# lmdu/pyfastx

Measured on AMD Instinct MI355X. Metric: FASTA index build + 1M random 100bp subseq fetches, 3 Gbp plain FASTA per GPU (throughput of the whole step, stream resident in HBM), higher is better.
Workload: dtype u8; 1 GPU; configs[1]: synthetic 3.0 Gbp hg38-shaped plain FASTA per GPU (200 contigs, 60-col LF, soft-masked, N runs), index build + 1000000 random 100 bp intervals (50% '-' strand); parallelism=one GPU, the whole stream resident in its HBM

## Files before the change

pyfastx_amd/csrc/fx_kernels.hpp:

```cpp
#pragma once
#include <hip/hip_runtime.h>
#include <stdint.h>

namespace fx {

constexpr int BLOCK = 256;
constexpr int UNROLL = 8;
constexpr int CHUNK = 16;
constexpr int TILE = BLOCK * CHUNK * UNROLL;

__device__ __forceinline__ uint32_t zero_bytes(uint32_t x) {
    return ~(((x & 0x7F7F7F7Fu) + 0x7F7F7F7Fu) | x | 0x7F7F7F7Fu);
}
__device__ __forceinline__ uint32_t flags4(uint32_t t) { return __builtin_amdgcn_udot4(t, 0x08040201u, 0u, false) >> 7; }
__device__ __forceinline__ uint32_t eq_mask16(const uint4 &v, uint32_t pat) {
    uint32_t lo = __builtin_amdgcn_udot4(zero_bytes(v.x ^ pat), 0x08040201u, 0u, false);
    lo = __builtin_amdgcn_udot4(zero_bytes(v.y ^ pat), 0x80402010u, lo, false);
    uint32_t hi = __builtin_amdgcn_udot4(zero_bytes(v.z ^ pat), 0x08040201u, 0u, false);
    hi = __builtin_amdgcn_udot4(zero_bytes(v.w ^ pat), 0x80402010u, hi, false);
    return (lo >> 7) | (hi << 1);
}

__device__ __forceinline__ uint4 load16(const uint8_t *__restrict__ data, int64_t p, int64_t n) {
    if (p + CHUNK <= n) return *reinterpret_cast<const uint4 *>(data + p);
// ... 327 lines not shown
                    uint32_t word = w[0];
#pragma unroll
                    for (int k = 1; k < NW; ++k) word = (j >> 2) == k ? w[k] : word;
                    uint8_t c = (uint8_t)(word >> ((j & 3) * 8));
                    if ((fl & 1) && c >= 'a' && c <= 'z') c -= 32;
                    if (fl & 4) c = lut[c];
                    const int64_t o = r - skip;
                    out[(fl & 2) ? (take - 1 - o) : o] = c;
                }
                ++r;
            }
            rank += total;
        }
        if (ok) {
            int64_t got = rank - skip;
            got = got < 0 ? 0 : (got > take ? take : got);
            if ((fl & 2) && got < take && got > 0) {
                const int64_t delta = take - got;
                for (int64_t j0 = 0; j0 < got; j0 += G) {
                    const int64_t j = j0 + sub;
                    uint8_t c = 0;
                    if (j < got) c = out[delta + j];
                    if (j < got) out[j] = c;
                }
            }
            if (sub == 0 && q.out_len) q.out_len[i] = got;
        }
    }
}

template <int G, int NP, bool COAL = false>
__global__ __launch_bounds__(BLOCK) void k_fetch_lines(const uint8_t *__restrict__ data, int64_t gbase, int64_t n_bytes, FetchQ q, FastaTab tab,
                                                      int64_t nq, int flags_all, uint8_t *__restrict__ dst, int32_t *__restrict__ list,
                                                      int *__restrict__ list_n) {
    __shared__ uint8_t lut[256];
    constexpr int CO_CAP = 2048;
    __shared__ __attribute__((aligned(16))) uint32_t s_out[COAL ? BLOCK / 64 : 1][COAL ? (CO_CAP + 32) / 4 : 1];
    constexpr int TABCAP = 512;
    __shared__ int64_t s_boff[TABCAP], s_slen[TABCAP];
    __shared__ int32_t s_llen[TABCAP], s_en[TABCAP];
    const int64_t n_seq = tab.n_seq_dev ? (*tab.n_seq_dev < tab.n_seq ? (int64_t)*tab.n_seq_dev : tab.n_seq) : tab.n_seq;
    const bool tab_lds = n_seq <= TABCAP && n_seq > 0;
    build_comp_lut(lut);
    if (tab_lds)
        for (int r = threadIdx.x; r < (int)n_seq; r += BLOCK) {
            s_boff[r] = tab.boff[r]; s_slen[r] = tab.slen[r];
            const int64_t ll = tab.llen[r];
            s_llen[r] = ll > 0x7FFFFFFFll ? 0x7FFFFFFF : (int32_t)ll;
            s_en[r] = tab.elen[r] | (tab.norm[r] << 8);
        }
    __syncthreads();
    constexpr int QPW = 64 / G;
    const int lane = lane_id(), sub = lane & (G - 1), grp = lane / G;
    const int64_t wave = ((int64_t)blockIdx.x * BLOCK + threadIdx.x) >> 6;
    const int64_t nwaves = ((int64_t)gridDim.x * BLOCK) >> 6;
    int64_t d_id = 0, d_a = 0, d_b = 0, d_off = 0;
    int d_fl = flags_all;
    auto fetch_desc = [&](int64_t i) {
        if (i >= nq) return;
        d_id = q.seq_id[i]; d_a = q.start[i]; d_b = q.stop[i];
        d_off = q.dst_off[i];
        d_fl = q.qflags ? q.qflags[i] : flags_all;
    };
    fetch_desc(wave * QPW + grp);
    for (int64_t i0 = wave * QPW; i0 < nq; i0 += nwaves * QPW) {
        const int64_t i = i0 + grp;
        const bool live = i < nq;
        const int64_t id = d_id, a = d_a, b = d_b;
// ... 339 lines not shown
```

pyfastx_amd/csrc/fx_spanscan.hpp:

```cpp
#pragma once
#include "fx_kernels.hpp"

namespace fx {

#ifndef FX_GRAN
#define FX_GRAN 4096
#endif
constexpr int GRAN = FX_GRAN;
constexpr int GR_ROWS = GRAN / (64 * CHUNK);
constexpr int SPAN_GRANS = 65536 / GRAN;
constexpr int SPAN = GRAN * SPAN_GRANS;
constexpr uint32_t SP_NONE = 0xFFFFFFFFu;

struct GranOut { uint32_t n, h, first, last, v1, c1, v2, c2, ovf; };
struct __attribute__((aligned(16))) GranPk { uint32_t nh, fl, d1, d2; };
__device__ __forceinline__ GranPk gran_pack(const GranOut &o) {
    GranPk p;
    p.nh = o.n | (o.h << 16); p.fl = (o.first & 0xFFFFu) | (o.last << 16);
    p.d1 = o.v1 | (o.c1 << 16); p.d2 = o.v2 | (o.c2 << 16) | (o.ovf << 31);
    return p;
}
__device__ __forceinline__ GranOut gran_unpack(const GranPk &p) {
    GranOut o;
    o.n = p.nh & 0xFFFFu; o.h = p.nh >> 16;
// ... 284 lines not shown
    }
    Tri tot;
    tri_block_incl(gran_tri(go, (int64_t)blockIdx.x * CG + threadIdx.x, ngran, gbase), lds, &tot);
    if (threadIdx.x == 0) ct[blockIdx.x] = ChunkTot{tot.n, tot.h, tot.last, 0};
}

struct Tri32 { uint32_t n, h; int32_t last; };
__device__ __forceinline__ Tri32 tri32_block_incl(Tri32 v, uint32_t (*lds)[16], Tri32 *total) {
    const int w = threadIdx.x >> 6, l = lane_id(), nw = (blockDim.x + 63) >> 6;
#pragma unroll
    for (int d = 1; d < 64; d <<= 1) {
        const uint32_t a = __shfl_up(v.n, d, 64), b = __shfl_up(v.h, d, 64);
        const int32_t c = __shfl_up(v.last, d, 64);
        if (l >= d) { v.n += a; v.h += b; v.last = c > v.last ? c : v.last; }
    }
    __syncthreads();
    if (l == 63) { lds[0][w] = v.n; lds[1][w] = v.h; lds[2][w] = (uint32_t)v.last; }
    __syncthreads();
    Tri32 base{0, 0, -1}, tot{0, 0, -1};
    for (int i = 0; i < nw; ++i) {
        const uint32_t a = lds[0][i], b = lds[1][i];
        const int32_t c = (int32_t)lds[2][i];
        if (i < w) { base.n += a; base.h += b; base.last = c > base.last ? c : base.last; }
        tot.n += a; tot.h += b; tot.last = c > tot.last ? c : tot.last;
    }
    *total = tot;
    return Tri32{base.n + v.n, base.h + v.h, base.last > v.last ? base.last : v.last};
}

template <int CG>
__global__ __launch_bounds__(CG) void k_gran_prefix(const GranPk *__restrict__ go, int64_t ngran, int64_t gbase,
                                                            const ChunkTot *__restrict__ ct, Totals *__restrict__ tot,
                                                            int64_t *__restrict__ nl_prefix, int64_t *__restrict__ hdr_prefix,
                                                            int64_t *__restrict__ prevnl) {
    __shared__ Tri lds[CG / 64];
    __shared__ uint32_t lds32[3][16];
    Tri b{0, 0, -1};
    for (int64_t c = threadIdx.x; c < (int64_t)blockIdx.x; c += CG) { const ChunkTot t = ct[c]; b = tri_join(b, Tri{t.n, t.h, t.last}); }
    Tri base{0, 0, -1};
    if (blockIdx.x) tri_block_incl(b, lds, &base);
    const int64_t g = (int64_t)blockIdx.x * CG + threadIdx.x;
    Tri32 v{0, 0, -1};
    if (g < ngran) {
        const GranOut o = gran_unpack(go[g]);
        v = Tri32{o.n, o.h, o.n ? (int32_t)(threadIdx.x * GRAN + o.last) : -1};
    }
    Tri32 total;
    const Tri32 inc = tri32_block_incl(v, lds32, &total);
    const int64_t cstart = gbase + (int64_t)blockIdx.x * CG * GRAN;
    if (g < ngran) {
        nl_prefix[g] = base.n + (inc.n - v.n);
        hdr_prefix[g] = base.h + (inc.h - v.h);
        int32_t pm = __shfl_up(inc.last, 1, 64);
        if (lane_id() == 0) { pm = -1; for (int i = 0; i < (int)(threadIdx.x >> 6); ++i) { const int32_t c = (int32_t)lds32[2][i]; pm = c > pm ? c : pm; } }
        prevnl[g] = pm >= 0 ? cstart + pm : base.last;
    }
    if (blockIdx.x == gridDim.x - 1 && threadIdx.x == 0) {
        const int64_t tn = base.n + total.n, th = base.h + total.h, tl = total.last >= 0 ? cstart + total.last : base.last;
        nl_prefix[ngran] = tn; hdr_prefix[ngran] = th; prevnl[ngran] = tl;
        tot->n_nl = tn; tot->n_hdr = th; tot->last_nl = tl;
    }
}

struct ScanCtx {
    const uint8_t *data; int64_t n, gbase, ngran;
    const GranPk *go;
    const int64_t *nl_prefix, *hdr_prefix, *prevnl;
};

__device__ __forceinline__ int64_t next_nl(const ScanCtx &c, int64_t x) {
    const int64_t y = x + 1 - c.gbase;
    if (y > c.n) return -1;
    const int64_t g = y / GRAN;
    if (g < c.ngran) {
        const GranOut o = gran_unpack(c.go[g]);
        const int64_t gs = g * (int64_t)GRAN;
        if (o.n && gs + o.last >= y) {
            if (gs + o.first >= y) return c.gbase + gs + o.first;
            for (int64_t p = y & ~(int64_t)(CHUNK - 1); p < gs + GRAN; p += CHUNK) {
                const uint4 v = load16(c.data, p, c.n);
                uint32_t m = eq_mask16(v, 0x0A0A0A0Au);
                if (p < y) m &= 0xFFFFu << (y - p);
                if (m) return c.gbase + p + (__ffs(m) - 1);
                if (p + CHUNK > c.n) break;
            }
            return c.gbase + gs + o.last;
        }
    }
    const int64_t key = c.gbase + (g + 1) * (int64_t)GRAN;
    int64_t lo = g + 1, hi = c.ngran;
    if (lo >= hi || c.prevnl[c.ngran] < key) return -1;
    while (lo < hi) { const int64_t mid = (lo + hi) >> 1; if (c.prevnl[mid + 1] >= key) hi = mid; else lo = mid + 1; }
    return c.gbase + lo * (int64_t)GRAN + (c.go[lo].fl & 0xFFFFu);
// ... 281 lines not shown
            if (mism) atomicAdd(&rv.bad[r], mism);
            return;
        }
    }
    irr.g[atomicAdd(irr.count, 1u)] = (uint32_t)g;
}

__global__ __launch_bounds__(BLOCK) void k_gran_exact(ScanCtx x, RecView rv, int64_t cap, GranList irr, int is_last, int prev_byte) {
    const int lane = lane_id();
    const int64_t wave = ((int64_t)blockIdx.x * blockDim.x + threadIdx.x) >> 6;
    const int64_t nwaves = ((int64_t)gridDim.x * blockDim.x) >> 6;
    const int64_t cnt = *irr.count;
    int64_t i = wave, g = i < cnt ? irr.g[i] : 0;
    uint4 v[GR_ROWS];
    if (i < cnt) {
#pragma unroll
        for (int j = 0; j < GR_ROWS; ++j) v[j] = load16(x.data, g * (int64_t)GRAN + j * 1024 + lane * CHUNK, x.n);
    }
    for (; i < cnt; i += nwaves) {
        const int64_t gc = g, hb = x.hdr_prefix[gc];
        int64_t he = x.hdr_prefix[gc + 1];
        if (he > cap) he = cap;
        ExactMasks mk;
        exact_masks(x, v, is_last, prev_byte, gc, he > hb, mk);
        if (i + nwaves < cnt) {
            g = irr.g[i + nwaves];
#pragma unroll
            for (int j = 0; j < GR_ROWS; ++j) v[j] = load16(x.data, g * (int64_t)GRAN + j * 1024 + lane * CHUNK, x.n);
        }
        exact_rows(x, rv, cap, gc, hb, mk);
    }
}

__global__ __launch_bounds__(BLOCK) void k_fasta_finalize2(int64_t cap, FastaCols c, Totals *__restrict__ tot,
                                                          const uint8_t *__restrict__ data, int64_t n_bytes, int64_t gbase) {
    const int64_t *__restrict__ hdr = c.hoff, *__restrict__ hdr_line = c.hdr_line;
    const int64_t k = (int64_t)blockIdx.x * BLOCK + threadIdx.x;
    const int64_t n_hdr = tot->n_hdr < cap ? tot->n_hdr : cap;
    int64_t s = 0;
    if (k < n_hdr) {
        if (c.dlen[k] >= 0) {
            int64_t hn, Ln;
            if (k + 1 < n_hdr) { hn = hdr[k + 1]; Ln = hdr_line[k + 1]; }
            else               { hn = tot->last_nl + 1; Ln = tot->n_nl; }
            const int64_t nseq = Ln - hdr_line[k] - 1;
            const int64_t blen = hn - c.boff[k];
            s = blen - (int64_t)c.elen[k] * nseq;
            c.blen[k] = blen; c.slen[k] = s;
            const int norm = c.bad[k] > 1 ? 0 : 1;
            c.norm[k] = norm;
            int reg = line_regular(data, n_bytes, gbase, c.boff[k], blen, s, nseq > 0 ? c.llen[k] : 0, c.elen[k], norm);
            if (reg < 0) reg = c.bad[k] == 0;
            c.reg[k] = reg;
        } else { c.blen[k] = 0; c.slen[k] = 0; c.norm[k] = 1; c.reg[k] = 0; }
    }
    __shared__ unsigned long long blk;
    if (threadIdx.x == 0) blk = 0;
    __syncthreads();
    s = wave_sum64(s);
    if (lane_id() == 0 && s) atomicAdd(&blk, (unsigned long long)s);
    __syncthreads();
    if (threadIdx.x == 0 && blk) atomicAdd((unsigned long long *)&tot->seq_len, blk);
}

__global__ __launch_bounds__(BLOCK) void k_line_regular(const uint8_t *__restrict__ data, int64_t n_bytes, int64_t gbase, int64_t n,
                                                       const int64_t *__restrict__ boff, const int64_t *__restrict__ blen,
                                                       const int64_t *__restrict__ slen, const int64_t *__restrict__ llen,
                                                       const int32_t *__restrict__ elen, const int32_t *__restrict__ norm,
                                                       int32_t *__restrict__ reg) {
    const int64_t k = (int64_t)blockIdx.x * BLOCK + threadIdx.x;
    if (k < n) reg[k] = line_regular(data, n_bytes, gbase, boff[k], blen[k], slen[k], llen[k], elen[k], norm[k]) > 0 ? 1 : 0;
}

__device__ __forceinline__ int64_t prev_nl_wave(const ScanCtx &x, int64_t p) {
    const int64_t y = (p - x.gbase < x.n) ? p - x.gbase : x.n;
    if (y <= 0) return -1;
    const int64_t g = (y - 1) / GRAN;
    const int64_t a = g * (int64_t)GRAN + lane_id() * 64;
    unsigned long long m = 0;
#pragma unroll
    for (int i = 0; i < 4; ++i)
        if (a + i * CHUNK < y) m |= (unsigned long long)eq_mask16(load16(x.data, a + i * CHUNK, x.n), 0x0A0A0A0Au) << (16 * i);
    if (y - a < 64) m &= (y - a <= 0) ? 0ull : (~0ull >> (64 - (y - a)));
    const unsigned long long b = __ballot(m != 0);
    if (!b) return x.prevnl[g];
    const int l = 63 - __clzll(b);
    const int hi = __shfl((int)(m >> 32), l, 64), lo = __shfl((int)(m & 0xFFFFFFFFull), l, 64);
    const unsigned long long ml = ((unsigned long long)(unsigned int)hi << 32) | (unsigned int)lo;
    return x.gbase + g * (int64_t)GRAN + l * 64 + (63 - __clzll(ml));
}

constexpr int SUMM_BLOCK = 1024;
__device__ __forceinline__ DiffSet diffset_shfl_xor(const DiffSet &d, int m) {
    return DiffSet{(uint32_t)__shfl_xor((int)d.v1, m, 64), (uint32_t)__shfl_xor((int)d.c1, m, 64), (uint32_t)__shfl_xor((int)d.v2, m, 64),
                   (uint32_t)__shfl_xor((int)d.c2, m, 64), (uint32_t)__shfl_xor((int)d.ovf, m, 64)};
// ... 210 lines not shown
```

pyfastx_amd/csrc/fxgpu.hip:

```cpp
#include <hip/hip_runtime.h>
#include <zlib.h>
#include <fcntl.h>
#include <pthread.h>
#include <sched.h>
#include <sys/mman.h>
#include <sys/stat.h>
#include <unistd.h>

#include <algorithm>
#include <atomic>
#include <chrono>
#include <functional>
#include <map>
#include <memory>
#include <cstdarg>
#include <cstdio>
#include <cstdlib>
#include <cstring>
#include <mutex>
#include <string>
#include <thread>
#include <vector>

#include "../../include/fxgpu.h"
// ... 313 lines not shown
        (h)->prof.end((h)->stream);                                               \
    } while (0)
#define FX_LAUNCH_LDS(h, id, kern, grid, block, lds, ...)                         \
    do {                                                                          \
        (h)->prof.begin(id, (h)->stream);                                         \
        hipLaunchKernelGGL(kern, grid, block, lds, (h)->stream, __VA_ARGS__);     \
        (h)->prof.end((h)->stream);                                               \
    } while (0)

struct StageAsync;
static void stage_drop(fx_handle *h);
struct fx_handle {
    int device = 0;
    hipStream_t stream = nullptr;
    StageAsync *stage = nullptr;
    int stage_fd = -1;
    hipStream_t stream2 = nullptr;
    uint8_t *d_data = nullptr;
    uint8_t *d_alloc = nullptr;
    size_t blob_cap = 0;
    bool owns = false;
    int64_t n = 0;
    bool gz = false;
    int64_t base = 0;
    int prev_byte = '\n';
    bool is_last = true;
    int64_t n_nl = 0;
    bool scanned = false;
    int64_t ngran = 0;
    DevBuf<GranPk> gran;
    DevBuf<uint32_t> hdr_grans, irr_grans;
    DevBuf<ChunkTot> chunks;
    DevBuf<unsigned long long> ctl;
    Totals *pin_tot = nullptr;
    struct OneBox { int64_t off, blen, skip, take, dst_off, out_len; } *one_box = nullptr;
    uint8_t *one_out = nullptr;
    Mailbox *mb = nullptr;
    hipStream_t mb_stream = nullptr;
    unsigned long long mb_seq = 0;
    bool mb_running = false, mb_off = false;
    DevBuf<uint32_t> nm_table;
    DevBuf<int64_t> nm_off;
    uint64_t nm_mask = 0;
    int nm_kind = -1;
    DevBuf<int64_t> nl_prefix, hdr_prefix, prevnl;
    DevBuf<int64_t> hdr, fa_boff, fa_blen, fa_slen, fa_llen, fa_hdr_line;
    DevBuf<int32_t> fa_elen, fa_norm, fa_dlen, fa_name_len, fa_reg;
    DevBuf<uint32_t> fa_bad;
    int64_t n_hdr = 0, fa_seqlen = 0;
    bool fasta_built = false;
    bool build_pending = false;
    int pending_full_name = 0;
    DevBuf<uint32_t> comp_runs;
    int comp_gpw = 0;
    bool comp_runs_valid = false;
    DevBuf<int64_t> fq_name_off, fq_rlen, fq_soff, fq_qoff;
    DevBuf<int32_t> fq_name_len, fq_dlen, fq_qlen;
    DevBuf<FastqAcc> fq_acc;
    DevBuf<FqRun> fq_runs;
    DevBuf<FastqAcc> fq_acc_build;
    DevBuf<uint32_t> fq_rej;
    int64_t fq_comp_runs = 0, fq_comp_rejected = 0;
    bool fq_comp_valid = false;
    int64_t fq_comp_base[5] = {0, 0, 0, 0, 0};
    int fq_comp_minqs = 104, fq_comp_maxqs = 33;
    DevBuf<uint32_t> fq_lines;
    bool fq_by_lines = false;
// ... 1520 lines not shown
        if (rc) return rc;
        for (int64_t i = 0; i < m; ++i) {
            unsigned char c = buf[i];
            if (!(c == ' ' || (c >= 9 && c <= 13))) { *out = c; return FX_OK; }
        }
    }
    return FX_OK;
}


static ScanCtx scan_ctx(const fx_handle *h) {
    ScanCtx x;
    x.data = h->d_data; x.n = h->n; x.gbase = h->base; x.ngran = h->ngran;
    x.go = h->gran.p; x.nl_prefix = h->nl_prefix.p; x.hdr_prefix = h->hdr_prefix.p; x.prevnl = h->prevnl.p;
    return x;
}
static FastaCols fasta_cols(fx_handle *h) {
    FastaCols c;
    c.hoff = h->hdr.p; c.boff = h->fa_boff.p; c.blen = h->fa_blen.p; c.slen = h->fa_slen.p; c.llen = h->fa_llen.p;
    c.hdr_line = h->fa_hdr_line.p; c.elen = h->fa_elen.p; c.dlen = h->fa_dlen.p; c.name_len = h->fa_name_len.p;
    c.norm = h->fa_norm.p; c.bad = h->fa_bad.p; c.reg = h->fa_reg.p;
    return c;
}
static int alloc_fasta_table(fx_handle *h, int64_t cap) {
    int rc;
    if ((rc = h->hdr.alloc(cap)) || (rc = h->fa_hdr_line.alloc(cap)) || (rc = h->fa_boff.alloc(cap)) ||
        (rc = h->fa_blen.alloc(cap)) || (rc = h->fa_slen.alloc(cap)) || (rc = h->fa_llen.alloc(cap)) ||
        (rc = h->fa_elen.alloc(cap)) || (rc = h->fa_norm.alloc(cap)) || (rc = h->fa_dlen.alloc(cap)) ||
        (rc = h->fa_name_len.alloc(cap)) || (rc = h->fa_bad.alloc(cap)) || (rc = h->fa_reg.alloc(cap)))
        return rc;
    return FX_OK;
}

static Totals *ctl_totals(fx_handle *h) { return (Totals *)h->ctl.p; }
static uint32_t *ctl_counter(fx_handle *h, int i) { return (uint32_t *)(h->ctl.p + 8 + i); }

static int comp_run_granules(int64_t ngran) {
    return ngran >= 65536 ? 4 * COMP_DEPTH : ngran >= 16384 ? 2 * COMP_DEPTH : COMP_DEPTH;
}

template <int MODE>
static int granule_pass(fx_handle *h, bool fq_lines = false, bool with_comp = false) {
    int rc;
    const int64_t nfull = h->n / GRAN, ngran = nfull + 1;
    const bool small = ngran <= (2ll << 20);
    const int64_t cg = small ? 256 : 1024, nchunks = (ngran + cg - 1) / cg;
    h->ngran = ngran;
    if ((rc = h->gran.alloc(ngran)) || (rc = h->hdr_grans.alloc(ngran)) || (MODE == 0 && (rc = h->irr_grans.alloc(ngran))) ||
        (rc = h->chunks.alloc(nchunks)) ||
        (rc = h->ctl.alloc(64)) || (rc = h->nl_prefix.alloc(ngran + 1)) || (rc = h->hdr_prefix.alloc(ngran + 1)) ||
        (rc = h->prevnl.alloc(ngran + 1)))
        return rc;
    if (!h->pin_tot) HIPCHK(hipHostMalloc((void **)&h->pin_tot, sizeof(Totals), hipHostMallocDefault));
    HIPCHK(hipMemsetAsync(h->ctl.p, 0, 64 * sizeof(unsigned long long), h->stream));
    GranList hgl{h->hdr_grans.p, ctl_counter(h, 0)};
    const int SCAN_WG = 512;
    if (nfull > 0 && MODE == 1 && fq_lines) {
        if ((rc = h->fq_lines.alloc((nfull + FQR_G - 1) / FQR_G * FQR_G * FQL_CAP))) return rc;
        if (with_comp) {
            const int64_t nruns = (nfull + FQLC_G - 1) / FQLC_G;
            if ((rc = h->fq_runs.alloc(nruns)) || (rc = h->fq_acc_build.alloc(1)) || (rc = h->fq_rej.alloc(nruns + 1))) return rc;
            static const int64_t grid_cap = [] { const char *e = getenv("FX_FQ_FUSED_GRID"); return e && atoll(e) > 0 ? atoll(e) : 6144ll; }();
            static const int force_crlf = [] { const char *e = getenv("FX_FQ_CRLF"); return e ? atoi(e) : -1; }();
            if (force_crlf >= 0 ? force_crlf != 0 : h->fq_crlf)
                FX_LAUNCH(h, K_FASTQ_LINES, k_fastq_lines_comp<true>, dim3((unsigned)std::min<int64_t>(nblocks(nruns, BLOCK / 64), grid_cap)), dim3(BLOCK), h->d_data,
                          h->n, h->prev_byte, nfull, h->gran.p, h->fq_lines.p, hgl, h->fq_runs.p, nruns);
            else
                FX_LAUNCH(h, K_FASTQ_LINES, k_fastq_lines_comp<false>, dim3((unsigned)std::min<int64_t>(nblocks(nruns, BLOCK / 64), grid_cap)), dim3(BLOCK), h->d_data,
                          h->n, h->prev_byte, nfull, h->gran.p, h->fq_lines.p, hgl, h->fq_runs.p, nruns);
        } else
        FX_LAUNCH(h, K_FASTQ_LINES, k_fastq_lines, dim3(nblocks(nfull, (BLOCK / 64) * FQL_G)), dim3(BLOCK), h->d_data, h->n, h->prev_byte, nfull,
                  h->gran.p, h->fq_lines.p, hgl);
    } else if (nfull > 0 && MODE == 0 && with_comp) {
        const int gpw = comp_run_granules(ngran);
        const int64_t runs = (ngran + gpw - 1) / gpw;
        if ((rc = h->comp_runs.alloc(runs * RUN_WORDS))) return rc;
        HIPCHK(hipMemsetAsync(h->comp_runs.p, 0, (size_t)runs * RUN_WORDS * 4, h->stream));
        FX_LAUNCH(h, K_SCAN_COMP, k_scan_comp, dim3(nblocks(runs, COMP_WPB)), dim3(COMP_WPB * 64), h->d_data, h->n, h->prev_byte,
                  (int)h->is_last, nfull, h->gran.p, hgl, gpw, h->comp_runs.p);
        h->comp_gpw = gpw;
        h->comp_runs_valid = true;
    } else if (nfull > 0)
        FX_LAUNCH(h, K_SPAN_SCAN, (k_span_scan<MODE>), dim3(nblocks((nfull + SCAN_GPW - 1) / SCAN_GPW * 64, SCAN_WG)), dim3(SCAN_WG), h->d_data, h->n,
                  h->prev_byte, (int)h->is_last, nfull, h->gran.p, hgl);
    if (small) {
        FX_LAUNCH(h, K_GRAN_REDUCE, (k_gran_reduce<MODE, 256>), dim3((unsigned)nchunks), dim3(256), h->d_data, h->n, h->prev_byte,
                  (int)h->is_last, hgl, h->gran.p, ngran, h->base, h->chunks.p);
        FX_LAUNCH(h, K_GRAN_PREFIX, (k_gran_prefix<256>), dim3((unsigned)nchunks), dim3(256), h->gran.p, ngran, h->base,
                  h->chunks.p, ctl_totals(h), h->nl_prefix.p, h->hdr_prefix.p, h->prevnl.p);
    } else {
        FX_LAUNCH(h, K_GRAN_REDUCE, (k_gran_reduce<MODE, 1024>), dim3((unsigned)nchunks), dim3(1024), h->d_data, h->n, h->prev_byte,
                  (int)h->is_last, hgl, h->gran.p, ngran, h->base, h->chunks.p);
        FX_LAUNCH(h, K_GRAN_PREFIX, (k_gran_prefix<1024>), dim3((unsigned)nchunks), dim3(1024), h->gran.p, ngran, h->base,
                  h->chunks.p, ctl_totals(h), h->nl_prefix.p, h->hdr_prefix.p, h->prevnl.p);
    }
    if (MODE == 1 && fq_lines && with_comp && nfull > 0) {
        FastqAcc init;
        memset(&init, 0, sizeof init);
        init.minqs = 104; init.maxqs = 33;
        HIPCHK(hipMemcpyAsync(h->fq_acc_build.p, &init, sizeof init, hipMemcpyHostToDevice, h->stream));
        const int64_t nruns = (nfull + FQLC_G - 1) / FQLC_G;
        HIPCHK(hipMemsetAsync(h->fq_rej.p, 0, 4, h->stream));
        FX_LAUNCH(h, K_FASTQ_COMP, k_fastq_comp_reduce, dim3((unsigned)std::min<int64_t>(nblocks(nruns, BLOCK), 1024)), dim3(BLOCK), (const FqRun *)h->fq_runs.p,
                  nruns, (const int64_t *)h->nl_prefix.p, (int64_t)0, h->d_data, h->n, nfull, h->fq_acc_build.p, h->fq_rej.p);
    }
    HIPCHK(hipGetLastError());
    return FX_OK;
}

static int enqueue_records(fx_handle *h, int full_name) {
    const ScanCtx x = scan_ctx(h);
    const int64_t cap = h->hdr.cap, ngran = h->ngran;
    const FastaCols c = fasta_cols(h);
    const RecView rv{h->fa_boff.p, h->fa_llen.p, h->fa_dlen.p, h->fa_bad.p, h->hdr.p};
    const GranList hgl{h->hdr_grans.p, ctl_counter(h, 0)}, irr{h->irr_grans.p, ctl_counter(h, 1)};
    FX_LAUNCH(h, K_HDR_REC, k_hdr_rec, dim3(2048), dim3(BLOCK), x, h->prev_byte, (int)h->is_last, full_name, hgl, c, cap);
    FX_LAUNCH(h, K_GRAN_LINES, k_gran_lines, dim3(nblocks(ngran, BLOCK)), dim3(BLOCK), x, rv, cap, irr);
    FX_LAUNCH(h, K_GRAN_EXACT, k_gran_exact, dim3(2048), dim3(BLOCK), x, rv, cap, irr, (int)h->is_last, h->prev_byte);
    FX_LAUNCH(h, K_FASTA_FINALIZE, k_fasta_finalize2, dim3(nblocks(cap, BLOCK)), dim3(BLOCK), cap, c, ctl_totals(h), h->d_data, h->n, h->base);
    HIPCHK(hipGetLastError());
    HIPCHK(hipMemcpyAsync(h->pin_tot, ctl_totals(h), sizeof(Totals), hipMemcpyDeviceToHost, h->stream));
    return FX_OK;
}

extern "C" int fx_fasta_build_begin(fx_handle *h, int full_name) {
    if (!h) return fail(FX_EINVAL, "null handle");
    int rc = use_device(h);
    if (rc) return rc;
    if (h->n <= 0) return fail(FX_EFORMAT, "empty input");
    h->scanned = false;
    h->nm_kind = -1;
    const bool with_comp = (full_name & 2) != 0;
    full_name &= 1;
    h->comp_runs_valid = h->rk_valid = false;
    if ((rc = granule_pass<0>(h, false, with_comp))) return rc;
    if (h->hdr.cap < 4096 && (rc = alloc_fasta_table(h, 4096))) return rc;
    if ((rc = enqueue_records(h, full_name))) return rc;
    h->build_pending = true;
    h->pending_full_name = full_name;
    h->fasta_built = true;
    return FX_OK;
}

static int finish_build(fx_handle *h) {
    if (!h->build_pending) return FX_OK;
    int rc = use_device(h);
    if (rc) return rc;
    Totals tot;
    for (;;) {
        HIPCHK(hipStreamSynchronize(h->stream));
        tot = *h->pin_tot;
        if (tot.n_hdr <= h->hdr.cap) break;
        if ((rc = alloc_fasta_table(h, tot.n_hdr + tot.n_hdr / 16 + 16))) return rc;
        HIPCHK(hipMemsetAsync(&ctl_totals(h)->seq_len, 0, 8, h->stream));
        HIPCHK(hipMemsetAsync(ctl_counter(h, 1), 0, 4, h->stream));
        if ((rc = enqueue_records(h, h->pending_full_name))) return rc;
    }
    h->build_pending = false;
    h->n_hdr = tot.n_hdr;
    h->n_nl = tot.n_nl;
    h->fa_seqlen = tot.seq_len;
    if (tot.n_hdr <= 0 && h->base == 0 && h->is_last) { h->fasta_built = false; return fail(FX_EFORMAT, "no FASTA header line ('>') found"); }
    return FX_OK;
}

extern "C" int fx_fasta_build_end(fx_handle *h, fx_fasta_summary *out) {
    if (!h) return fail(FX_EINVAL, "null handle");
    if (!h->fasta_built) return fail(FX_ESTATE, "fx_fasta_build_begin has not run");
    int rc = finish_build(h);
    if (rc) return rc;
    if (out) { out->n_seq = h->n_hdr; out->seq_len = h->fa_seqlen; out->n_lines = h->n_nl; out->n_bytes = h->n; }
    return FX_OK;
}

extern "C" int fx_fasta_build(fx_handle *h, int full_name, fx_fasta_summary *out) {
    int rc = fx_fasta_build_begin(h, full_name);
    if (rc) return rc;
    return fx_fasta_build_end(h, out);
}

extern "C" int fx_fasta_set_table(fx_handle *h, int64_t n, const int64_t *boff, const int64_t *blen, const int64_t *slen,
                                  const int64_t *llen, const int32_t *elen, const int32_t *norm) {
    if (!h || n < 0 || (n > 0 && (!boff || !blen || !slen || !llen || !elen || !norm))) return fail(FX_EINVAL, "bad argument");
    int rc = use_device(h);
    if (rc) return rc;
    h->rk_valid = false;
    if ((rc = alloc_fasta_table(h, std::max<int64_t>(n, 1)))) return rc;
// ... 118 lines not shown
    if (where != FX_DEVICE) {
        if ((rc = out.alloc(3 * count))) return rc;
        ds = out.p; da = out.p + count; dn = out.p + 2 * count;
    }
    const unsigned nb = (unsigned)std::min<int64_t>(nblocks(n, BLOCK / 64), 2048);
    hipLaunchKernelGGL(k_comp_emit, dim3(nb), dim3(BLOCK), 0, h->stream, dense.p, n, off.p, ds, da, dn);
    HIPCHK(hipGetLastError());
    if (where != FX_DEVICE) {
        if ((rc = to_host(h, seqid, ds, count * 8)) || (rc = to_host(h, abc, da, count * 8)) || (rc = to_host(h, num, dn, count * 8))) return rc;
    }
    HIPCHK(hipStreamSynchronize(h->stream));
    return FX_OK;
}

extern "C" int fx_fasta_comp(fx_handle *h, int where, int64_t *comp) { return fasta_comp_impl(h, where, comp, -1, nullptr); }

extern "C" int fx_fasta_comp_shard(fx_handle *h, int where, int64_t *comp, int64_t lead_from, int64_t *lead) {
    if (!lead) return fail(FX_EINVAL, "null argument");
    return fasta_comp_impl(h, where, comp, lead_from, lead);
}

static int fastq_count(fx_handle *h, int64_t *n_nl_core, int64_t *last_nl_core, bool want_comp = false) {
    int rc = use_device(h);
    if (rc) return rc;
    if (h->n <= 0) return fail(FX_EFORMAT, "empty input");
    h->fasta_built = h->fastq_built = h->comp_runs_valid = h->rk_valid = false;
    h->fq_comp_valid = false;
    static const int force = [] { const char *e = getenv("FX_FQ_LINES"); return e ? atoi(e) : -1; }();
    bool by_lines = force > 0;
    h->fq_crlf = false;
    memset(g_build_laps, 0, sizeof g_build_laps);
    LapClock lc;
    if (h->n >= 4 * GRAN) {
        if ((rc = h->ctl.alloc(64))) return rc;
        HIPCHK(hipMemsetAsync(h->ctl.p + 56, 0, 3 * sizeof(unsigned long long), h->stream));
        hipLaunchKernelGGL(k_nl_sample, dim3(3), dim3(BLOCK), 0, h->stream, h->d_data, h->n, h->ctl.p + 56);
        HIPCHK(hipGetLastError());
        unsigned long long smp[3];
        HIPCHK(hipMemcpyAsync(smp, h->ctl.p + 56, sizeof smp, hipMemcpyDeviceToHost, h->stream));
        HIPCHK(hipStreamSynchronize(h->stream));
        if (force < 0) by_lines = smp[1] > 0 && (double)smp[0] / (double)smp[1] * GRAN <= 0.7 * FQL_CAP;
        h->fq_crlf = smp[2] > 0;
    }
    static const bool no_fuse = [] { const char *e = getenv("FX_FQ_NO_FUSED_COMP"); return e && atoi(e) != 0; }();
    const bool with_comp = want_comp && by_lines && !no_fuse && h->base == 0 && h->halo == 0 && h->is_last && h->n >= GRAN;
    lc.lap(0);
    if ((rc = granule_pass<1>(h, by_lines, with_comp))) return rc;
    lc.lap(1);
    int64_t *res = (int64_t *)(h->ctl.p + 48);
    hipLaunchKernelGGL(k_core_count, dim3(1), dim3(64), 0, h->stream, scan_ctx(h), (int)h->is_last, h->n - h->halo, res);
    HIPCHK(hipGetLastError());
    int64_t host[3];
    HIPCHK(hipMemcpyAsync(h->pin_tot, ctl_totals(h), sizeof(Totals), hipMemcpyDeviceToHost, h->stream));
    HIPCHK(hipMemcpyAsync(host, res, sizeof host, hipMemcpyDeviceToHost, h->stream));
    uint32_t n_over = 0;
    if (by_lines) HIPCHK(hipMemcpyAsync(&n_over, ctl_counter(h, 0), sizeof n_over, hipMemcpyDeviceToHost, h->stream));
    FastqAcc built;
    memset(&built, 0, sizeof built);
    uint32_t n_rej = 0;
    if (with_comp) {
        HIPCHK(hipMemcpyAsync(&built, h->fq_acc_build.p, sizeof built, hipMemcpyDeviceToHost, h->stream));
        HIPCHK(hipMemcpyAsync(&n_rej, h->fq_rej.p, 4, hipMemcpyDeviceToHost, h->stream));
    }
    HIPCHK(hipStreamSynchronize(h->stream));
    lc.lap(2);
    if (with_comp) {
        const int64_t nfull = h->n / GRAN, nruns = (nfull + FQLC_G - 1) / FQLC_G;
// ... 480 lines not shown
            h->pin_in_used += padded;
        }
        hipError_t e = hipMemcpyAsync(d, from, (size_t)bytes, hipMemcpyHostToDevice, h->stream);
        if (e != hipSuccess) return fail(FX_EDEVICE, "H2D: %s", hipGetErrorString(e));
        *dst = (const T *)d;
        return FX_OK;
    }
    template <class T> int scratch(int64_t n, T **dst) {
        void *d = take(n * (int64_t)sizeof(T));
        if (!d) return fail(FX_ENOMEM, "device scratch allocation failed");
        *dst = (T *)d;
        return FX_OK;
    }
};

static unsigned fetch_grid(int64_t nq) {
    static const int64_t cap = []() { const char *e = getenv("FX_FETCH_WG"); const int64_t v = e ? atoll(e) : 0; return v > 0 ? v : (int64_t)256 * 8 * 4; }();
    return (unsigned)std::max<int64_t>(1, std::min<int64_t>((nq + 3) / 4, cap));
}

static int fetch_launch(fx_handle *h, Staged &st, const FetchQ &q, bool by_id, bool longq, int64_t n, int flags, uint8_t *d_dst) {
    int rc;
    FastaTab tab;
    memset(&tab, 0, sizeof tab);
    if (h->fasta_built) {
        tab.boff = h->fa_boff.p; tab.blen = h->fa_blen.p; tab.slen = h->fa_slen.p; tab.llen = h->fa_llen.p;
        tab.elen = h->fa_elen.p; tab.norm = h->fa_reg.p; tab.n_seq = h->n_hdr;
        if (h->build_pending) { tab.n_seq_dev = (const long long *)&ctl_totals(h)->n_hdr; tab.n_seq = h->hdr.cap; }
    }
    static const int fetch_g = [] { const char *e = getenv("FX_FETCH_G"); return e ? atoi(e) : 4; }();
    static const bool lean = [] { const char *e = getenv("FX_FETCH_LEAN"); return !e || atoi(e) != 0; }();
    if (!longq && by_id && fetch_g == 4 && lean && n < 0x7FFFFFFFll) {
        int32_t *d_list = nullptr;
        int *d_cnt = nullptr;
        if ((rc = st.scratch<int32_t>(n, &d_list)) || (rc = st.scratch<int>(1, &d_cnt))) return rc;
        HIPCHK(hipMemsetAsync(d_cnt, 0, sizeof(int), h->stream));
        static const int np = [] { const char *e = getenv("FX_FETCH_NP"); return e ? atoi(e) : 1; }();
        static const bool coal = [] { const char *e = getenv("FX_FETCH_COAL"); return e && atoi(e) != 0; }();
        if (np == 1 && coal) FX_LAUNCH(h, K_FETCH, (k_fetch_lines<4, 1, true>), dim3(fetch_grid((n + 15) / 16)), dim3(BLOCK), h->d_data, h->base, h->n, q, tab, n, flags, d_dst, d_list, d_cnt);
        else if (np == 1) FX_LAUNCH(h, K_FETCH, (k_fetch_lines<4, 1>), dim3(fetch_grid((n + 15) / 16)), dim3(BLOCK), h->d_data, h->base, h->n, q, tab, n, flags, d_dst, d_list, d_cnt);
        else         FX_LAUNCH(h, K_FETCH, (k_fetch_lines<4, 2>), dim3(fetch_grid((n + 15) / 16)), dim3(BLOCK), h->d_data, h->base, h->n, q, tab, n, flags, d_dst, d_list, d_cnt);
        FX_LAUNCH(h, K_FETCH_REST, (k_fetch<true, 4, 16>), dim3(std::min(fetch_grid((n + 15) / 16), 1024u)), dim3(BLOCK), h->d_data, h->base, h->n, q, tab, n, flags,
                  d_dst, (const int32_t *)d_list, (const int *)d_cnt);
    } else if (!longq && by_id && fetch_g == 4) {
        FX_LAUNCH(h, K_FETCH, (k_fetch<true, 4, 16>), dim3(fetch_grid((n + 15) / 16)), dim3(BLOCK), h->d_data, h->base, h->n, q, tab, n, flags, d_dst);
    } else if (!longq && by_id && fetch_g == 2) {
        FX_LAUNCH(h, K_FETCH, (k_fetch<true, 2, 16>), dim3(fetch_grid((n + 31) / 32)), dim3(BLOCK), h->d_data, h->base, h->n, q, tab, n, flags, d_dst);
    } else if (!longq && by_id && fetch_g == 16) {
        FX_LAUNCH(h, K_FETCH, (k_fetch<true, 16, 16>), dim3(fetch_grid((n + 3) / 4)), dim3(BLOCK), h->d_data, h->base, h->n, q, tab, n, flags, d_dst);
    } else if (!longq) {
        const unsigned grid8 = fetch_grid((n + 7) / 8);
        if (by_id) FX_LAUNCH(h, K_FETCH, (k_fetch<true, 8, 16>), dim3(grid8), dim3(BLOCK), h->d_data, h->base, h->n, q, tab, n, flags, d_dst);
        else       FX_LAUNCH(h, K_FETCH, (k_fetch<false, 8, 16>), dim3(grid8), dim3(BLOCK), h->d_data, h->base, h->n, q, tab, n, flags, d_dst);
    } else {
        const unsigned grid = fetch_grid(n);
        if (by_id) FX_LAUNCH(h, K_FETCH, (k_fetch<true, 64, 16>), dim3(grid), dim3(BLOCK), h->d_data, h->base, h->n, q, tab, n, flags, d_dst);
        else       FX_LAUNCH(h, K_FETCH, (k_fetch<false, 64, 16>), dim3(grid), dim3(BLOCK), h->d_data, h->base, h->n, q, tab, n, flags, d_dst);
    }
    HIPCHK(hipGetLastError());
    return FX_OK;
}

static int fetch_common(fx_handle *h, int where, int64_t n, bool by_id, const int64_t *a0, const int64_t *a1,
                        const int64_t *a2, const int64_t *skip, int flags, const uint8_t *qflags, uint8_t *dst,
                        const int64_t *dst_off, int64_t *out_len, int64_t dst_bytes_hint) {
    if (!h) return fail(FX_EINVAL, "null handle");
    if (n < 0 || (n > 0 && (!a0 || !a1 || !a2 || !dst || !dst_off))) return fail(FX_EINVAL, "null query array");
    if (by_id && !h->fasta_built) return fail(FX_ESTATE, "fx_fasta_build has not run");
    if (n == 0) return FX_OK;
    int rc = use_device(h);
    if (rc) return rc;
    Staged st(h);
    FetchQ q;
    memset(&q, 0, sizeof q);
    const int64_t *host_blen = (where == FX_HOST && !by_id) ? a1 : nullptr;
    uint8_t *d_dst = dst;
// ... 3919 lines not shown
```

Baseline: 4924 Gbp/s.

## Remove per-pass memsets and D2H copy via double-buffered device counters

Replaces the per-build hipMemsetAsync of control words with generation double-buffering: each kernel clears the other generation's counters for the next pass. The finalize kernel now counts finished blocks with a ticket, and the last block writes totals straight into pinned host memory tagged with a sequence number, replacing a separate hipMemcpyAsync. The fetch path likewise alternates two list counters, with the fetch kernel zeroing the spare one, so the per-call memset goes away. The aim is fewer small stream operations and launches per step. The cost is subtler correctness, since it relies on system-scope fences and on redo flags to recover from error paths.

Result: no change. 4969 Gbp/s (median of 5 runs) (+0.9%).

```diff
diff --git a/pyfastx_amd/csrc/fx_kernels.hpp b/pyfastx_amd/csrc/fx_kernels.hpp
--- a/pyfastx_amd/csrc/fx_kernels.hpp
+++ b/pyfastx_amd/csrc/fx_kernels.hpp
@@ -383,8 +383,9 @@
 template <int G, int NP, bool COAL = false>
 __global__ __launch_bounds__(BLOCK) void k_fetch_lines(const uint8_t *__restrict__ data, int64_t gbase, int64_t n_bytes, FetchQ q, FastaTab tab,
                                                       int64_t nq, int flags_all, uint8_t *__restrict__ dst, int32_t *__restrict__ list,
-                                                      int *__restrict__ list_n) {
+                                                      int *__restrict__ list_n, int *__restrict__ clear_n) {
     __shared__ uint8_t lut[256];
+    if (blockIdx.x == 0 && threadIdx.x == 0) *clear_n = 0;
     constexpr int CO_CAP = 2048;
     __shared__ __attribute__((aligned(16))) uint32_t s_out[COAL ? BLOCK / 64 : 1][COAL ? (CO_CAP + 32) / 4 : 1];
     constexpr int TABCAP = 512;
diff --git a/pyfastx_amd/csrc/fx_spanscan.hpp b/pyfastx_amd/csrc/fx_spanscan.hpp
--- a/pyfastx_amd/csrc/fx_spanscan.hpp
+++ b/pyfastx_amd/csrc/fx_spanscan.hpp
@@ -340,7 +340,7 @@
 __global__ __launch_bounds__(CG) void k_gran_prefix(const GranPk *__restrict__ go, int64_t ngran, int64_t gbase,
                                                             const ChunkTot *__restrict__ ct, Totals *__restrict__ tot,
                                                             int64_t *__restrict__ nl_prefix, int64_t *__restrict__ hdr_prefix,
-                                                            int64_t *__restrict__ prevnl) {
+                                                            int64_t *__restrict__ prevnl, unsigned long long *__restrict__ other_gen) {
     __shared__ Tri lds[CG / 64];
     __shared__ uint32_t lds32[3][16];
     Tri b{0, 0, -1};
@@ -367,6 +367,7 @@
         const int64_t tn = base.n + total.n, th = base.h + total.h, tl = total.last >= 0 ? cstart + total.last : base.last;
         nl_prefix[ngran] = tn; hdr_prefix[ngran] = th; prevnl[ngran] = tl;
         tot->n_nl = tn; tot->n_hdr = th; tot->last_nl = tl;
+        other_gen[0] = 0; other_gen[1] = 0; other_gen[2] = 0; other_gen[3] = 0;
     }
 }
 
@@ -714,8 +715,9 @@
     }
 }
 
-__global__ __launch_bounds__(BLOCK) void k_fasta_finalize2(int64_t cap, FastaCols c, Totals *__restrict__ tot,
-                                                          const uint8_t *__restrict__ data, int64_t n_bytes, int64_t gbase) {
+__global__ __launch_bounds__(BLOCK) void k_fasta_finalize2(int64_t cap, FastaCols c, Totals *tot,
+                                                          const uint8_t *__restrict__ data, int64_t n_bytes, int64_t gbase,
+                                                          unsigned long long *acc, uint32_t *ticket, Totals *pin, long long seq) {
     const int64_t *__restrict__ hdr = c.hoff, *__restrict__ hdr_line = c.hdr_line;
     const int64_t k = (int64_t)blockIdx.x * BLOCK + threadIdx.x;
     const int64_t n_hdr = tot->n_hdr < cap ? tot->n_hdr : cap;
@@ -742,7 +744,19 @@
     s = wave_sum64(s);
     if (lane_id() == 0 && s) atomicAdd(&blk, (unsigned long long)s);
     __syncthreads();
-    if (threadIdx.x == 0 && blk) atomicAdd((unsigned long long *)&tot->seq_len, blk);
+    if (threadIdx.x == 0) {
+        if (blk) atomicAdd(acc, blk);
+        __threadfence();
+        if (atomicAdd(ticket, 1u) == gridDim.x - 1) {
+            __threadfence();
+            const long long sl = (long long)atomicAdd(acc, 0ull);
+            tot->seq_len = sl;
+            volatile Totals *p = pin;
+            p->n_nl = tot->n_nl; p->n_hdr = tot->n_hdr; p->last_nl = tot->last_nl; p->seq_len = sl;
+            __threadfence_system();
+            p->pad0 = seq;
+        }
+    }
 }
 
 __global__ __launch_bounds__(BLOCK) void k_line_regular(const uint8_t *__restrict__ data, int64_t n_bytes, int64_t gbase, int64_t n,
diff --git a/pyfastx_amd/csrc/fxgpu.hip b/pyfastx_amd/csrc/fxgpu.hip
--- a/pyfastx_amd/csrc/fxgpu.hip
+++ b/pyfastx_amd/csrc/fxgpu.hip
@@ -369,7 +369,13 @@
     DevBuf<uint32_t> hdr_grans, irr_grans;
     DevBuf<ChunkTot> chunks;
     DevBuf<unsigned long long> ctl;
+    int ctl_gen = 1;
+    bool ctl_redo = false;
     Totals *pin_tot = nullptr;
+    long long tot_seq = 0;
+    DevBuf<int> fetch_cnt;
+    unsigned fetch_no = 0;
+    bool fetch_cnt_redo = true;
     struct OneBox { int64_t off, blen, skip, take, dst_off, out_len; } *one_box = nullptr;
     uint8_t *one_out = nullptr;
     Mailbox *mb = nullptr;
@@ -1956,8 +1962,22 @@
     return FX_OK;
 }
 
+constexpr int CTL_GEN0 = 8, CTL_GEN_WORDS = 4;
 static Totals *ctl_totals(fx_handle *h) { return (Totals *)h->ctl.p; }
-static uint32_t *ctl_counter(fx_handle *h, int i) { return (uint32_t *)(h->ctl.p + 8 + i); }
+static unsigned long long *ctl_gen_words(fx_handle *h, int gen) { return h->ctl.p + CTL_GEN0 + CTL_GEN_WORDS * gen; }
+static uint32_t *ctl_counter(fx_handle *h, int i) { return (uint32_t *)(ctl_gen_words(h, h->ctl_gen) + i); }
+static unsigned long long *ctl_seq_acc(fx_handle *h) { return ctl_gen_words(h, h->ctl_gen) + 2; }
+static uint32_t *ctl_ticket(fx_handle *h) { return (uint32_t *)(ctl_gen_words(h, h->ctl_gen) + 3); }
+static int ctl_ready(fx_handle *h) {
+    const bool fresh = !h->ctl.p;
+    int rc = h->ctl.alloc(64);
+    if (rc) return rc;
+    if (fresh || h->ctl_redo) {
+        HIPCHK(hipMemsetAsync(h->ctl.p, 0, 64 * sizeof(unsigned long long), h->stream));
+        h->ctl_redo = false;
+    }
+    return FX_OK;
+}
 
 static int comp_run_granules(int64_t ngran) {
     return ngran >= 65536 ? 4 * COMP_DEPTH : ngran >= 16384 ? 2 * COMP_DEPTH : COMP_DEPTH;
@@ -1972,11 +1992,16 @@
     h->ngran = ngran;
     if ((rc = h->gran.alloc(ngran)) || (rc = h->hdr_grans.alloc(ngran)) || (MODE == 0 && (rc = h->irr_grans.alloc(ngran))) ||
         (rc = h->chunks.alloc(nchunks)) ||
-        (rc = h->ctl.alloc(64)) || (rc = h->nl_prefix.alloc(ngran + 1)) || (rc = h->hdr_prefix.alloc(ngran + 1)) ||
+        (rc = ctl_ready(h)) || (rc = h->nl_prefix.alloc(ngran + 1)) || (rc = h->hdr_prefix.alloc(ngran + 1)) ||
         (rc = h->prevnl.alloc(ngran + 1)))
         return rc;
-    if (!h->pin_tot) HIPCHK(hipHostMalloc((void **)&h->pin_tot, sizeof(Totals), hipHostMallocDefault));
-    HIPCHK(hipMemsetAsync(h->ctl.p, 0, 64 * sizeof(unsigned long long), h->stream));
+    if (!h->pin_tot) {
+        HIPCHK(hipHostMalloc((void **)&h->pin_tot, sizeof(Totals), hipHostMallocDefault));
+        memset(h->pin_tot, 0, sizeof(Totals));
+    }
+    h->ctl_gen ^= 1;
+    h->ctl_redo = true;
+    unsigned long long *const other_gen = ctl_gen_words(h, h->ctl_gen ^ 1);
     GranList hgl{h->hdr_grans.p, ctl_counter(h, 0)};
     const int SCAN_WG = 512;
     if (nfull > 0 && MODE == 1 && fq_lines) {
@@ -2011,12 +2036,12 @@
         FX_LAUNCH(h, K_GRAN_REDUCE, (k_gran_reduce<MODE, 256>), dim3((unsigned)nchunks), dim3(256), h->d_data, h->n, h->prev_byte,
                   (int)h->is_last, hgl, h->gran.p, ngran, h->base, h->chunks.p);
         FX_LAUNCH(h, K_GRAN_PREFIX, (k_gran_prefix<256>), dim3((unsigned)nchunks), dim3(256), h->gran.p, ngran, h->base,
-                  h->chunks.p, ctl_totals(h), h->nl_prefix.p, h->hdr_prefix.p, h->prevnl.p);
+                  h->chunks.p, ctl_totals(h), h->nl_prefix.p, h->hdr_prefix.p, h->prevnl.p, other_gen);
     } else {
         FX_LAUNCH(h, K_GRAN_REDUCE, (k_gran_reduce<MODE, 1024>), dim3((unsigned)nchunks), dim3(1024), h->d_data, h->n, h->prev_byte,
                   (int)h->is_last, hgl, h->gran.p, ngran, h->base, h->chunks.p);
         FX_LAUNCH(h, K_GRAN_PREFIX, (k_gran_prefix<1024>), dim3((unsigned)nchunks), dim3(1024), h->gran.p, ngran, h->base,
-                  h->chunks.p, ctl_totals(h), h->nl_prefix.p, h->hdr_prefix.p, h->prevnl.p);
+                  h->chunks.p, ctl_totals(h), h->nl_prefix.p, h->hdr_prefix.p, h->prevnl.p, other_gen);
     }
     if (MODE == 1 && fq_lines && with_comp && nfull > 0) {
         FastqAcc init;
@@ -2029,6 +2054,7 @@
                   nruns, (const int64_t *)h->nl_prefix.p, (int64_t)0, h->d_data, h->n, nfull, h->fq_acc_build.p, h->fq_rej.p);
     }
     HIPCHK(hipGetLastError());
+    h->ctl_redo = false;
     return FX_OK;
 }
 
@@ -2041,9 +2067,9 @@
     FX_LAUNCH(h, K_HDR_REC, k_hdr_rec, dim3(2048), dim3(BLOCK), x, h->prev_byte, (int)h->is_last, full_name, hgl, c, cap);
     FX_LAUNCH(h, K_GRAN_LINES, k_gran_lines, dim3(nblocks(ngran, BLOCK)), dim3(BLOCK), x, rv, cap, irr);
     FX_LAUNCH(h, K_GRAN_EXACT, k_gran_exact, dim3(2048), dim3(BLOCK), x, rv, cap, irr, (int)h->is_last, h->prev_byte);
-    FX_LAUNCH(h, K_FASTA_FINALIZE, k_fasta_finalize2, dim3(nblocks(cap, BLOCK)), dim3(BLOCK), cap, c, ctl_totals(h), h->d_data, h->n, h->base);
+    FX_LAUNCH(h, K_FASTA_FINALIZE, k_fasta_finalize2, dim3(nblocks(cap, BLOCK)), dim3(BLOCK), cap, c, ctl_totals(h), h->d_data, h->n, h->base,
+              ctl_seq_acc(h), ctl_ticket(h), h->pin_tot, ++h->tot_seq);
     HIPCHK(hipGetLastError());
-    HIPCHK(hipMemcpyAsync(h->pin_tot, ctl_totals(h), sizeof(Totals), hipMemcpyDeviceToHost, h->stream));
     return FX_OK;
 }
 
@@ -2074,9 +2100,11 @@
     for (;;) {
         HIPCHK(hipStreamSynchronize(h->stream));
         tot = *h->pin_tot;
+        if (tot.pad0 != h->tot_seq)
+            return fail(FX_EDEVICE, "the totals of record pass %lld did not arrive (pinned copy holds those of pass %lld)", h->tot_seq, tot.pad0);
         if (tot.n_hdr <= h->hdr.cap) break;
         if ((rc = alloc_fasta_table(h, tot.n_hdr + tot.n_hdr / 16 + 16))) return rc;
-        HIPCHK(hipMemsetAsync(&ctl_totals(h)->seq_len, 0, 8, h->stream));
+        HIPCHK(hipMemsetAsync(ctl_seq_acc(h), 0, 2 * sizeof(unsigned long long), h->stream));
         HIPCHK(hipMemsetAsync(ctl_counter(h, 1), 0, 4, h->stream));
         if ((rc = enqueue_records(h, h->pending_full_name))) return rc;
     }
@@ -2261,7 +2289,7 @@
     memset(g_build_laps, 0, sizeof g_build_laps);
     LapClock lc;
     if (h->n >= 4 * GRAN) {
-        if ((rc = h->ctl.alloc(64))) return rc;
+        if ((rc = ctl_ready(h))) return rc;
         HIPCHK(hipMemsetAsync(h->ctl.p + 56, 0, 3 * sizeof(unsigned long long), h->stream));
         hipLaunchKernelGGL(k_nl_sample, dim3(3), dim3(BLOCK), 0, h->stream, h->d_data, h->n, h->ctl.p + 56);
         HIPCHK(hipGetLastError());
@@ -2808,16 +2836,20 @@
     static const bool lean = [] { const char *e = getenv("FX_FETCH_LEAN"); return !e || atoi(e) != 0; }();
     if (!longq && by_id && fetch_g == 4 && lean && n < 0x7FFFFFFFll) {
         int32_t *d_list = nullptr;
-        int *d_cnt = nullptr;
-        if ((rc = st.scratch<int32_t>(n, &d_list)) || (rc = st.scratch<int>(1, &d_cnt))) return rc;
-        HIPCHK(hipMemsetAsync(d_cnt, 0, sizeof(int), h->stream));
+        if ((rc = st.scratch<int32_t>(n, &d_list)) || (rc = h->fetch_cnt.alloc(2))) return rc;
+        if (h->fetch_cnt_redo) HIPCHK(hipMemsetAsync(h->fetch_cnt.p, 0, 2 * sizeof(int), h->stream));
+        h->fetch_cnt_redo = true;
+        int *const d_cnt = h->fetch_cnt.p + (h->fetch_no & 1), *const d_clr = h->fetch_cnt.p + (~h->fetch_no & 1);
+        ++h->fetch_no;
         static const int np = [] { const char *e = getenv("FX_FETCH_NP"); return e ? atoi(e) : 1; }();
         static const bool coal = [] { const char *e = getenv("FX_FETCH_COAL"); return e && atoi(e) != 0; }();
-        if (np == 1 && coal) FX_LAUNCH(h, K_FETCH, (k_fetch_lines<4, 1, true>), dim3(fetch_grid((n + 15) / 16)), dim3(BLOCK), h->d_data, h->base, h->n, q, tab, n, flags, d_dst, d_list, d_cnt);
-        else if (np == 1) FX_LAUNCH(h, K_FETCH, (k_fetch_lines<4, 1>), dim3(fetch_grid((n + 15) / 16)), dim3(BLOCK), h->d_data, h->base, h->n, q, tab, n, flags, d_dst, d_list, d_cnt);
-        else         FX_LAUNCH(h, K_FETCH, (k_fetch_lines<4, 2>), dim3(fetch_grid((n + 15) / 16)), dim3(BLOCK), h->d_data, h->base, h->n, q, tab, n, flags, d_dst, d_list, d_cnt);
+        if (np == 1 && coal) FX_LAUNCH(h, K_FETCH, (k_fetch_lines<4, 1, true>), dim3(fetch_grid((n + 15) / 16)), dim3(BLOCK), h->d_data, h->base, h->n, q, tab, n, flags, d_dst, d_list, d_cnt, d_clr);
+        else if (np == 1) FX_LAUNCH(h, K_FETCH, (k_fetch_lines<4, 1>), dim3(fetch_grid((n + 15) / 16)), dim3(BLOCK), h->d_data, h->base, h->n, q, tab, n, flags, d_dst, d_list, d_cnt, d_clr);
+        else         FX_LAUNCH(h, K_FETCH, (k_fetch_lines<4, 2>), dim3(fetch_grid((n + 15) / 16)), dim3(BLOCK), h->d_data, h->base, h->n, q, tab, n, flags, d_dst, d_list, d_cnt, d_clr);
         FX_LAUNCH(h, K_FETCH_REST, (k_fetch<true, 4, 16>), dim3(std::min(fetch_grid((n + 15) / 16), 1024u)), dim3(BLOCK), h->d_data, h->base, h->n, q, tab, n, flags,
                   d_dst, (const int32_t *)d_list, (const int *)d_cnt);
+        HIPCHK(hipGetLastError());
+        h->fetch_cnt_redo = false;
     } else if (!longq && by_id && fetch_g == 4) {
         FX_LAUNCH(h, K_FETCH, (k_fetch<true, 4, 16>), dim3(fetch_grid((n + 15) / 16)), dim3(BLOCK), h->d_data, h->base, h->n, q, tab, n, flags, d_dst);
     } else if (!longq && by_id && fetch_g == 2) {
```
